# siboehm/ShallowSpeed

Measured on AMD Instinct MI355X. Metric: samples/sec (whole node), 4-layer MLP MNIST-shape, DP×PP at 1/2/4/8 GPUs, higher is better.
Workload: dtype bf16; 1 GPU; model=mlp4_mnist_784x256x256x256x10, global_batch=16384, parallelism=dp1, schedule=naive, loss=xent, mubatches=1, hipgraph=False, fp8_fwd=False, deterministic=False

## Files before the change

### csrc/bindings.cpp

```cpp

#include <torch/extension.h>

#include <ATen/cuda/CUDAContext.h>

#include <climits>
#include <optional>
#include <string>

#include "launchers.h"

namespace {

hipStream_t cur_stream() {
    return (hipStream_t)at::cuda::getCurrentCUDAStream().stream();
}

void check_bf16(const torch::Tensor& t, const char* name) {
    TORCH_CHECK(t.is_cuda(), name, " must be on GPU");
    TORCH_CHECK(t.scalar_type() == torch::kBFloat16, name, " must be bf16");
    TORCH_CHECK(t.is_contiguous(), name, " must be contiguous");
}

void check_f32(const torch::Tensor& t, const char* name) {
    TORCH_CHECK(t.is_cuda(), name, " must be on GPU");
// ... 187 lines not shown
        out = {torch::empty({M, N}, a.options().dtype(torch::kBFloat16))};
        ok = ss_gemm_nt_f8(a.data_ptr(), asc.data_ptr(), b.data_ptr(),
                           bsc.data_ptr(), bias_p, out[0].data_ptr(), M, N, K,
                           relu, cur_stream());
    }
    TORCH_CHECK(ok, "shape outside the fp8 tier: ", M, "x", N, "x", K);
    return out;
}

torch::Tensor gemm_nt_f8(torch::Tensor a, torch::Tensor asc, torch::Tensor b,
                         torch::Tensor bsc, torch::Tensor bias, bool relu) {
    return gemm_nt_f8_any(false, a, asc, b, bsc, bias, relu)[0];
}

std::vector<torch::Tensor> gemm_nt_f8_q(torch::Tensor a, torch::Tensor asc,
                                         torch::Tensor b, torch::Tensor bsc,
                                         torch::Tensor bias, bool relu) {
    return gemm_nt_f8_any(true, a, asc, b, bsc, bias, relu);
}

void wgrad_tn_256(torch::Tensor dy, torch::Tensor x, torch::Tensor gw) {
    check_bf16(dy, "dy");
    check_bf16(x, "x");
    check_f32(gw, "gw");
    const int Kb = dy.size(0), Mo = dy.size(1), N = x.size(1);
    TORCH_CHECK(x.size(0) == Kb, "batch mismatch");
    TORCH_CHECK(gw.size(0) == Mo && gw.size(1) == N, "gw shape");
    TORCH_CHECK(ss_wgrad_tn_256(dy.data_ptr(), x.data_ptr(), gw.data_ptr(),
                                Mo, N, Kb, cur_stream()),
                "shape outside the 256-tile wgrad tier");
}

void wgrad_tn(torch::Tensor dy, torch::Tensor x, torch::Tensor gw,
              torch::Tensor gb, torch::Tensor mask, int64_t split_k) {
    check_bf16(dy, "dy");
    check_bf16(x, "x");
    check_f32(gw, "gw");
    const int Kb = dy.size(0), Mo = dy.size(1), N = x.size(1);
    TORCH_CHECK(x.size(0) == Kb, "batch mismatch");
    TORCH_CHECK(gw.size(0) == Mo && gw.size(1) == N, "gw shape");
    const void* mask_p = opt_bf16(mask, "mask");
    TORCH_CHECK(!mask_p || mask.sizes() == dy.sizes(), "mask must match dy");
    void* gb_p = opt_f32(gb, "gb");
    TORCH_CHECK(!gb_p || gb.numel() == Mo, "gb size");
    ss_wgrad_tn(dy.data_ptr(), x.data_ptr(), mask_p, gw.data_ptr(), gb_p, Mo,
                N, Kb, (int)split_k, cur_stream());
}

void wgrad_tn_multi(torch::Tensor chunk_table, int64_t nchunks,
                    bool has_mask, torch::Tensor gw, torch::Tensor gb,
                    int64_t Mo, int64_t N, int64_t kb_chunk,
                    int64_t split_k) {
    check_table(chunk_table, 3, "chunk_table must be CUDA int64 [nchunks,3]");
    TORCH_CHECK(chunk_table.size(0) == nchunks,
                "chunk_table must be CUDA int64 [nchunks,3]");
    check_f32(gw, "gw");
    TORCH_CHECK(gw.size(0) == Mo && gw.size(1) == N, "gw shape");
    void* gb_p = opt_f32(gb, "gb");
    TORCH_CHECK(!gb_p || gb.numel() == Mo, "gb size");
    ss_wgrad_tn_multi(chunk_table.data_ptr(), (int)nchunks, has_mask,
                      gw.data_ptr(), gb_p, (int)Mo, (int)N, (int)kb_chunk,
                      (int)split_k, cur_stream());
}

torch::Tensor colsum(torch::Tensor dy, torch::Tensor mask) {
    check_bf16(dy, "dy");
    const void* mask_p = opt_bf16(mask, "mask");
    auto gb = torch::zeros({dy.size(1)},
                           dy.options().dtype(torch::kFloat));
    ss_colsum(dy.data_ptr(), mask_p, gb.data_ptr(), dy.size(0), dy.size(1),
              cur_stream());
    return gb;
}

torch::Tensor relu_fwd(torch::Tensor x, std::optional<torch::Tensor> out) {
    check_bf16(x, "x");
    auto y = out_like(x, out);
    ss_relu_fwd(x.data_ptr(), y.data_ptr(), x.numel(), cur_stream());
    return y;
// ... 392 lines not shown
                                 out.data_ptr(), cur_stream()),
                "shape outside the fused-MLP tier");
    return out;
}

void transpose_bf16(torch::Tensor src, torch::Tensor dst) {
    check_bf16(src, "src");
    check_bf16(dst, "dst");
    const int rows = src.size(0), cols = src.size(1);
    TORCH_CHECK(src.dim() == 2 && dst.dim() == 2 &&
                    dst.size(0) == cols && dst.size(1) == rows &&
                    rows % 64 == 0 && cols % 64 == 0,
                "transpose_bf16 needs 64-aligned 2-D shapes");
    ss_transpose_bf16(src.data_ptr(), dst.data_ptr(), rows, cols,
                      cur_stream());
}

}

PYBIND11_MODULE(TORCH_EXTENSION_NAME, m) {
    m.def("gemm_nt", &gemm_nt, "C = A @ B^T (+bias)(+relu) with optional A-mask");
    m.def("gemm_nt_256", &gemm_nt_256,
          "256-tile 8-phase GEMM (M%256==N%256==K%128==0)");
    m.def("gemm_nt_256w", &gemm_nt_256w,
          "256-tile 8-phase GEMM, 4-wave 128x128-wave-tile variant");
    m.def("wgrad_tn_256", &wgrad_tn_256,
          "256-tile 8-phase wgrad: gw += dy^T @ x (no mask/bias)");
    m.def("fp8_quantize", &fp8_quantize,
          "bf16 [R,K] -> (e4m3 u8 [R,K], e8m0 scales [K/128,R,4])");
    m.def("gemm_nt_f8", &gemm_nt_f8,
          "MX-fp8 256-tile GEMM: C=bf16(A@B^T) (+bias)(+relu)");
    m.def("gemm_nt_f8_q", &gemm_nt_f8_q,
          "MX-fp8 GEMM with FUSED output quantization -> (e4m3, scales)");
    m.def("wgrad_tn", &wgrad_tn, "gW += (dy⊙mask)^T @ x; gb += colsum (fused)");
    m.def("colsum", &colsum, "standalone column sum (bias grad)");
    m.def("wgrad_tn_multi", &wgrad_tn_multi,
          "chunked (deferred-µbatch) wgrad: one launch, many (dy,x) pairs");
    m.def("relu_fwd", &relu_fwd, py::arg("x"), py::arg("out") = py::none());
    m.def("relu_bwd", &relu_bwd, py::arg("dy"), py::arg("y"),
          py::arg("out") = py::none());
    m.def("relu_bwd_scaled", &relu_bwd_scaled,
          "dz = bf16(dy * scale) where y > 0, else +0", py::arg("dy"),
          py::arg("y"), py::arg("scale"), py::arg("out") = py::none());
    m.def("gemm_nt_dropout", &gemm_nt_dropout,
          "C = dropout(relu(A @ B^T + bias)), mask in the GEMM epilogue",
          py::arg("a"), py::arg("b"), py::arg("bias"), py::arg("key0"),
          py::arg("key1"), py::arg("step"), py::arg("layer"),
          py::arg("row_first"), py::arg("row_stride"), py::arg("thr"),
          py::arg("scale"), py::arg("fused") = true);
    m.def("dropout_fwd_", &dropout_fwd_,
          "in-place dropout of a finished post-ReLU activation");
    m.def("dropout_keep_mask", &dropout_keep_mask,
          "keep bits (bool [M][ncols]) for explicit sample ids");
    m.def("softmax_fwd", &softmax_fwd);
    m.def("softmax_bwd", &softmax_bwd);
    m.def("head_mse_bwd", &head_mse_bwd);
    m.def("head_xent_bwd", &head_xent_bwd, py::arg("probs"),
          py::arg("target"), py::arg("global_batch"),
          py::arg("out") = py::none());
    m.def("head_fwd_fused", &head_fwd_fused,
          "fused head forward: softmax(bf16(x @ w^T + b))", py::arg("x"),
          py::arg("w"), py::arg("b"), py::arg("rows_per_block") = 0);
    m.def("head_bwd_fused", &head_bwd_fused,
          "fused head backward -> (dz, dx); optional gW/gb accumulate",
          py::arg("probs"), py::arg("target"), py::arg("x"), py::arg("w_t"),
          py::arg("global_batch"), py::arg("grad_w"), py::arg("grad_b"),
          py::arg("rows_per_block") = 0,
// ... 34 lines not shown
```

### csrc/launchers.h

```cpp
#pragma once

#include <hip/hip_runtime.h>

#include <cstdint>

inline bool aligned16(const void* p) { return p && ((uintptr_t)p & 15) == 0; }

void ss_gemm_nt(const void* A, const void* B, const void* bias,
                const void* mask, void* C, int M, int N, int K, bool relu,
                hipStream_t stream);
void ss_colsum(const void* dY, const void* mask, void* gb, int M, int N,
               hipStream_t stream);

struct DropoutArgs {
    unsigned key0, key1;
    unsigned layer, step;
    unsigned row_first, row_stride;
    unsigned thr;
    float scale;
};
bool ss_gemm_nt_dropout(const void* A, const void* B, const void* bias,
                        void* C, int M, int N, int K,
                        const DropoutArgs& drop, hipStream_t stream);

bool ss_gemm_nt_256(const void* A, const void* B, const void* bias, void* C,
                    int M, int N, int K, bool relu, hipStream_t stream);
bool ss_gemm_nt_256w(const void* A, const void* B, const void* bias, void* C,
                     int M, int N, int K, bool relu, hipStream_t stream);

void ss_fp8_quantize(const void* X, void* Q, void* S, int R, int K,
                     hipStream_t stream);
bool ss_gemm_nt_f8(const void* A, const void* Asc, const void* B,
                   const void* Bsc, const void* bias, void* C, int M, int N,
                   int K, bool relu, hipStream_t stream);
bool ss_gemm_nt_f8_q(const void* A, const void* Asc, const void* B,
                     const void* Bsc, const void* bias, void* Cq, void* Cs,
                     int M, int N, int K, bool relu, hipStream_t stream);

void ss_wgrad_tn(const void* dY, const void* X, const void* mask, void* gW,
                 void* gb, int Mo, int N, int Kb, int split_k,
                 hipStream_t stream);
void ss_wgrad_tn_multi(const void* chunk_table, int nchunks, bool has_mask,
                       void* gW, void* gb, int Mo, int N, int Kb_chunk,
                       int split_k, hipStream_t stream);
bool ss_wgrad_tn_256(const void* dY, const void* X, void* gW, int Mo, int N,
                     int Kb, hipStream_t stream);

bool ss_head_fwd_fused(const void* x, const void* W, const void* bias,
                       void* probs, int M, int K, int C, int rows_per_block,
                       hipStream_t stream);
bool ss_head_bwd_fused(const void* probs, const void* target, const void* x,
                       const void* Wt, void* dz, void* dx, void* gW, void* gb,
                       int M, int K, int C, float inv_gb, int rows_per_block,
                       void* metrics, int slots, hipStream_t stream);
bool ss_head_metrics(const void* probs, const void* target, void* acc,
                     int slots, int M, int C, int kind, hipStream_t stream);

constexpr int SS_BWD_CHAIN_MAX = 8;
bool ss_bwd_chain(const void* probs, const void* target, const void* Wt_head,
                  void* dz_head, const void* const* h, const void* const* wt,
                  void* const* dz, int nlayers, void* dx, int M, int H, int C,
                  float inv_gb, int rows, int waves, int w_lds,
                  float dz_scale, hipStream_t stream);

constexpr int SS_FWD_CHAIN_MAX = 8;
bool ss_fwd_chain(const void* x, const void* const* w, const void* const* b,
                  void* const* h, int nlayers, const void* W_head,
                  const void* b_head, void* probs, int M, int K0, int H, int C,
                  int rows, int waves, int l1, hipStream_t stream);

bool ss_fused_mlp_fwd(const void* x, const void* desc, int M, int in_dim,
                      int nhidden, int cout, void* out, hipStream_t stream);

// ... 46 lines not shown
```

### csrc/wgrad.hip

```cpp

#include "common.h"
#include "launchers.h"

using gbf16 = __attribute__((address_space(1))) __bf16;
using gbf16x8 = __attribute__((address_space(1))) bf16x8;

template <int BMT, int BNT, bool HAS_MASK, int KG>
__global__ __launch_bounds__(KG * 256, BMT* BNT > 64 * 64 ? 2 : 4)
void wgrad_tn_kernel(
    const __bf16* __restrict__ dY,
    const __bf16* __restrict__ X,
    const __bf16* __restrict__ mask,
    float* __restrict__ gW,
    float* __restrict__ gb,
    int Mo, int N, int Kb, int k_per_split,
    const long* __restrict__ chunks, int nsplit) {
    constexpr int BKW = 64;
    constexpr int NMA = BMT / 16;
    constexpr int NMB = BNT / 16;
    constexpr int FM = BMT / 32;
    constexpr int FN = BNT / 32;
    constexpr int NT = KG * 256;
    constexpr int A_EL = NMA * 16 * 64;
    constexpr int B_EL = NMB * 16 * 64;
    constexpr int GRP_EL = A_EL + B_EL;
    constexpr int STAGE_F = KG * GRP_EL / 2;
    constexpr int NPASS = BMT * BNT <= STAGE_F       ? 1
                          : BMT * BNT <= 2 * STAGE_F ? 2
                                                     : 4;
    constexpr int RP = BMT / NPASS;
    static_assert(RP % 16 == 0 && RP * BNT <= STAGE_F, "epilogue band");
    static_assert(KG * 256 <= STAGE_F, "bias partials fit the staging");

    __shared__ __attribute__((aligned(16))) ushort smem[KG * GRP_EL];

    const int tid = threadIdx.x;
    const int lane = tid & 63;
    const int gtid = tid & 255;
    const int wv = __builtin_amdgcn_readfirstlane(tid >> 6);
    const int wave = wv & 3;
    const int grp = wv >> 2;
    const int wm = wave >> 1;
    const int wn = wave & 1;
    ushort* const At = smem + grp * GRP_EL;
    ushort* const Bt = At + A_EL;
    const int gx = gridDim.x, gy = gridDim.y;
    const int nwg = gx * gy * gridDim.z;
    const int hw = blockIdx.x + gx * (blockIdx.y + gy * blockIdx.z);
    const int wid = xcd_remap(hw, nwg);
    const int bidy = wid % gy;
    const int bidx = (wid / gy) % gx;
    int bidz = wid / (gy * gx);
    if (chunks) {
        const long* row = chunks + (long)(bidz / nsplit) * 3;
        dY = (const __bf16*)row[0];
        X = (const __bf16*)row[1];
        mask = (const __bf16*)row[2];
        bidz = bidz % nsplit;
    }
    const gbf16* const gdY = (const gbf16*)dY;
    const gbf16* const gX = (const gbf16*)X;
    const gbf16* const gmask = (const gbf16*)mask;
    const int m0 = bidx * BMT;
    const int n0 = bidy * BNT;
    const int kbeg = bidz * k_per_split;
    const int kend = min(Kb, kbeg + k_per_split);

    f32x4 acc[FM][FN];
#pragma unroll
    for (int i = 0; i < FM; ++i)
#pragma unroll
        for (int j = 0; j < FN; ++j) acc[i][j] = {0.f, 0.f, 0.f, 0.f};

    const int fmv = min(FM, max(0, (Mo - m0 - wm * (BMT / 2) + 15) / 16));
    const int fnv = min(FN, max(0, (N - n0 - wn * (BNT / 2) + 15) / 16));

    const bool do_db = (gb != nullptr) && (bidy == 0);
    float db_part = 0.f;

    auto swsub = [](int ksub) {
        return (ksub & ~3) | ((ksub & 1) << 1) | ((ksub >> 1) & 1);
    };
    auto baddr = [swsub](int k, int m) {
        return ((m >> 4) * 16 + swsub(k >> 2)) * 64 + (k & 3) * 16 + (m & 15);
    };

    constexpr int ELA = BKW * BMT / 256;
    constexpr int ELB = BKW * BNT / 256;
    constexpr int CA = ELA / 8, CB = ELB / 8;
    const int ska = (gtid * ELA) / BMT, sma = (gtid * ELA) % BMT;
    const int skb = (gtid * ELB) / BNT, smb = (gtid * ELB) % BNT;
    bf16x8 ra[CA], rmk[CA], rb[CB];

    auto load_chunk = [](const gbf16* p, const gbf16* base, int valid,
                         auto width_mult8) {
        bf16x8 v;
        if constexpr (decltype(width_mult8)::value) {
            v = *(const gbf16x8*)(valid > 0 ? p : base);
            return v;
        }
#pragma unroll
        for (int i = 0; i < 8; ++i) v[i] = (__bf16)0.f;
        if (valid >= 8) {
            v = *(const gbf16x8*)p;
        } else if (valid > 0) {
#pragma unroll
            for (int i = 0; i < 8; ++i) {
                const __bf16 t = p[i < valid ? i : 0];
                v[i] = i < valid ? t : (__bf16)0.f;
            }
        }
        return v;
    };
    const bool vecA = (Mo & 7) == 0, vecB = (N & 7) == 0;
    auto left_a = [&](int k0) {
        return k0 + ska < kend ? Mo - (m0 + sma) : 0;
    };
    auto left_b = [&](int k0) {
        return k0 + skb < kend ? N - (n0 + smb) : 0;
    };
    auto stage_load = [&](int k0) {
        {
            const long off = (long)(k0 + ska) * Mo + m0 + sma;
            const int left = left_a(k0);
            auto rows = [&](auto w8) {
#pragma unroll
                for (int ch = 0; ch < CA; ++ch) {
                    ra[ch] = load_chunk(gdY + off + ch * 8, gdY,
                                        left - ch * 8, w8);
                    if constexpr (HAS_MASK)
                        rmk[ch] = load_chunk(gmask + off + ch * 8, gmask,
                                             left - ch * 8, w8);
                }
            };
            if (vecA) {
                rows(std::true_type{});
            } else {
                rows(std::false_type{});
                __builtin_amdgcn_s_waitcnt(0x0F70);
            }
        }
        {
            const long off = (long)(k0 + skb) * N + n0 + smb;
            const int left = left_b(k0);
            auto rows = [&](auto w8) {
#pragma unroll
                for (int ch = 0; ch < CB; ++ch)
                    rb[ch] = load_chunk(gX + off + ch * 8, gX, left - ch * 8,
                                        w8);
            };
            if (vecB) {
                rows(std::true_type{});
            } else {
                rows(std::false_type{});
                __builtin_amdgcn_s_waitcnt(0x0F70);
            }
        }
    };
    auto stage_write = [&](int k0) {
        const int la = left_a(k0), lb = left_b(k0);
#pragma unroll
        for (int ch = 0; ch < CA; ++ch) {
            bf16x8 v = ra[ch];
            const bool in = la - ch * 8 > 0;
#pragma unroll
            for (int i = 0; i < 8; ++i) {
                bool keep = in;
                if constexpr (HAS_MASK)
                    keep = keep && bf2f(rmk[ch][i]) > 0.f;
                if (!keep) v[i] = (__bf16)0.f;
            }
            *(bf16x8*)&At[baddr(ska, sma + ch * 8)] = v;
        }
#pragma unroll
        for (int ch = 0; ch < CB; ++ch) {
            bf16x8 v = rb[ch];
            if (!(lb - ch * 8 > 0)) {
#pragma unroll
                for (int i = 0; i < 8; ++i) v[i] = (__bf16)0.f;
            }
            *(bf16x8*)&Bt[baddr(skb, smb + ch * 8)] = v;
        }
    };

    auto glds_stage = [&](const gbf16* src, ushort* img,
                          int nmt, int ld, int base_col, int gk0) {
        const int total = nmt * 16 * 8;
        const int per_wave = total / 4;
        for (int i0 = 0; i0 < per_wave; i0 += 64) {
            const int q = wave * per_wave + i0 + lane;
            const int p = q >> 3, rr = q & 7;
            const int ksub = ((p & 15) & ~3) | (((p & 15) & 1) << 1) |
                             (((p & 15) >> 1) & 1);
            const int k = ksub * 4 + (rr >> 1);
            const int m = (p >> 4) * 16 + (rr & 1) * 8;
            __builtin_amdgcn_global_load_lds(
                (gptr_t)(src + (long)(gk0 + k) * ld + base_col + m),
                (lptr_t)(img + (long)(wave * per_wave + i0) * 8), 16, 0,
                0);
        }
    };
    auto full_tile = [&](int k0) {
        return !HAS_MASK && m0 + BMT <= Mo && n0 + BNT <= N &&
               k0 + BKW <= kend;
    };

    const int lcol4 = (lane & 15) * 4;
    auto mma_step = [&](auto all_cols) {
        constexpr int FNU = decltype(all_cols)::value ? FN : 1;
#pragma unroll
        for (int kk = 0; kk < BKW / 32; ++kk) {
            const int g2 = kk * 8 + (lane >> 4) * 2;
            bf16x8 a_frag[FM], b_frag[FNU];
#pragma unroll
            for (int i = 0; i < FM; ++i) {
                const int mblk = wm * FM + i;
                bf16x4v lo = __builtin_amdgcn_ds_read_tr16_b64_v4bf16(
                    (lds_v4p)&At[(mblk * 16 + swsub(g2)) * 64 + lcol4]);
                bf16x4v hi = __builtin_amdgcn_ds_read_tr16_b64_v4bf16(
                    (lds_v4p)&At[(mblk * 16 + swsub(g2 + 1)) * 64 + lcol4]);
#pragma unroll
                for (int e = 0; e < 4; ++e) {
                    a_frag[i][e] = lo[e];
                    a_frag[i][e + 4] = hi[e];
                }
            }
#pragma unroll
            for (int j = 0; j < FNU; ++j) {
                const int nblk = wn * FN + j;
                bf16x4v lo = __builtin_amdgcn_ds_read_tr16_b64_v4bf16(
                    (lds_v4p)&Bt[(nblk * 16 + swsub(g2)) * 64 + lcol4]);
                bf16x4v hi = __builtin_amdgcn_ds_read_tr16_b64_v4bf16(
                    (lds_v4p)&Bt[(nblk * 16 + swsub(g2 + 1)) * 64 + lcol4]);
#pragma unroll
                for (int e = 0; e < 4; ++e) {
                    b_frag[j][e] = lo[e];
                    b_frag[j][e + 4] = hi[e];
                }
            }
#pragma unroll
            for (int i = 0; i < FM; ++i) {
#pragma unroll
                for (int j = 0; j < FNU; ++j)
                    acc[i][j] = __builtin_amdgcn_mfma_f32_16x16x32_bf16(
                        a_frag[i], b_frag[j], acc[i][j], 0, 0, 0);
            }
        }
    };

    const int nsteps = kend > kbeg ? (kend - kbeg + BKW - 1) / BKW : 0;
    const int niter = (nsteps + KG - 1) / KG;
    int k0 = kbeg + grp * BKW;
    if (k0 < kend && !full_tile(k0)) stage_load(k0);
    for (int it = 0; it < niter; ++it, k0 += KG * BKW) {
        const bool active = k0 < kend;
        __builtin_amdgcn_s_waitcnt(0x0F70);
        if (active) {
            if (full_tile(k0)) {
                glds_stage(gdY, At, NMA, Mo, m0, k0);
                glds_stage(gX, Bt, NMB, N, n0, k0);
            } else {
                stage_write(k0);
            }
        }
        __syncthreads();

        const int kn = k0 + KG * BKW;
        if (kn < kend && !full_tile(kn)) stage_load(kn);

        if (active) {
            if (do_db) {
                constexpr int NKQ = 256 / BMT;
                constexpr int KPT = BKW / NKQ;
                const int m = gtid % BMT, kq = gtid / BMT;
#pragma unroll
                for (int j = 0; j < KPT; ++j) {
                    const ushort u = At[baddr(kq * KPT + j, m)];
                    db_part += bf2f(*(const __bf16*)&u);
                }
            }
            if (fmv > 0 && fnv > 1)
                mma_step(std::true_type{});
            else if (fmv > 0 && fnv == 1)
                mma_step(std::false_type{});
        }
        __syncthreads();
    }

    float* const red = (float*)smem;

    if (do_db) {
        constexpr int NQ = KG * (256 / BMT);
        red[tid] = db_part;
        __syncthreads();
        if (tid < BMT && m0 + tid < Mo) {
            float s = 0.f;
#pragma unroll
            for (int qq = 0; qq < NQ; ++qq) s += red[qq * BMT + tid];
            atomicAdd(&gb[m0 + tid], s);
        }
        __syncthreads();
    }

    const int lrow = lane & 15;
    const int kch = lane >> 4;
#pragma unroll
    for (int p = 0; p < NPASS; ++p) {
#pragma unroll
        for (int g = 0; g < KG; ++g) {
            if (grp == g) {
#pragma unroll
                for (int i = 0; i < FM; ++i) {
                    const int trow = wm * (BMT / 2) + i * 16;
                    if (trow / RP != p || i >= fmv) continue;
#pragma unroll
                    for (int j = 0; j < FN; ++j) {
                        if (j >= fnv) continue;
                        const int cc = wn * (BNT / 2) + j * 16 + lrow;
#pragma unroll
                        for (int rr = 0; rr < 4; ++rr) {
                            const int ix =
                                (trow - p * RP + kch * 4 + rr) * BNT + cc;
                            if (g == 0)
                                red[ix] = acc[i][j][rr];
                            else
                                red[ix] += acc[i][j][rr];
                        }
                    }
                }
            }
            __syncthreads();
        }
        for (int ix = tid; ix < RP * BNT; ix += NT) {
            const int grow = m0 + p * RP + ix / BNT;
            const int gcol = n0 + ix % BNT;
            if (grow < Mo && gcol < N)
                atomicAdd(&gW[(long)grow * N + gcol], red[ix]);
        }
        if (p + 1 < NPASS) __syncthreads();
    }
}


namespace {

constexpr int WGRAD_KG_128 = 2;
constexpr int WGRAD_KG_64 = 4;
constexpr int WGRAD_TARGET_BLOCKS = 256;

struct WgradCfg {
    int bm, bn, kg;
};

WgradCfg wgrad_cfg(int Mo, int N, int split_k) {
    int tile = ((Mo >= 256 && N >= 512) || (Mo >= 512 && N >= 256)) ? 1 : 0;
    static const int env_big = env_int("SS_WGRAD_BIG", -1);
    static const int env_kg = env_int("SS_WGRAD_KG", -1);
    if (env_big >= 0) tile = env_big > 2 ? 1 : env_big;
    WgradCfg c;
    c.bm = tile == 1 ? 128 : 64;
    c.bn = tile == 0 ? 64 : 128;
    c.kg = tile == 0 ? WGRAD_KG_64 : WGRAD_KG_128;
    if (env_kg == 1 || env_kg == 2 || env_kg == 4) c.kg = env_kg;
    if (tile != 0 && c.kg > 2) c.kg = 2;
    if (split_k == 1) c.kg = 1;
    return c;
}

int wgrad_auto_split(int tiles, int Kb, int kg) {
    static const int env_blocks = env_int("SS_WGRAD_BLOCKS", 0);
    const int target = env_blocks > 0 ? env_blocks : WGRAD_TARGET_BLOCKS;
    int split_k = cdiv(target, tiles);
    while (split_k & (split_k - 1)) split_k &= split_k - 1;
    const int max_split = cdiv(Kb, 64 * kg);
    if (split_k > max_split) split_k = max_split;
    return split_k;
}

}

#define WGRAD_LAUNCH(BMT, BNT, HM, KGV, ...)                                \
    hipLaunchKernelGGL((wgrad_tn_kernel<BMT, BNT, HM, KGV>), grid,          \
                       dim3(KGV * 256), 0, stream, __VA_ARGS__)
#define WGRAD_BY_MASK(BMT, BNT, KGV, ...)                                   \
    do {                                                                    \
        if (has_mask) WGRAD_LAUNCH(BMT, BNT, true, KGV, __VA_ARGS__);       \
        else WGRAD_LAUNCH(BMT, BNT, false, KGV, __VA_ARGS__);               \
    } while (0)
#define WGRAD_DISPATCH(cfg, ...)                                            \
    do {                                                                    \
        if (cfg.bm == 128) {                                                \
            if (cfg.kg == 1) WGRAD_BY_MASK(128, 128, 1, __VA_ARGS__);       \
            else WGRAD_BY_MASK(128, 128, 2, __VA_ARGS__);                   \
        } else if (cfg.bn == 128) {                                         \
            if (cfg.kg == 1) WGRAD_BY_MASK(64, 128, 1, __VA_ARGS__);        \
            else WGRAD_BY_MASK(64, 128, 2, __VA_ARGS__);                    \
        } else {                                                            \
            if (cfg.kg == 1) WGRAD_BY_MASK(64, 64, 1, __VA_ARGS__);         \
            else if (cfg.kg == 2) WGRAD_BY_MASK(64, 64, 2, __VA_ARGS__);    \
            else WGRAD_BY_MASK(64, 64, 4, __VA_ARGS__);                     \
        }                                                                   \
    } while (0)

void ss_wgrad_tn(const void* dY, const void* X, const void* mask, void* gW,
                 void* gb, int Mo, int N, int Kb, int split_k,
                 hipStream_t stream) {
    if (!mask && split_k <= 0 && Mo >= 512 && N >= 512 &&
        (long)(Mo / 256) * (N / 256) >= 64) {
        static const int en = env_int("SS_WGRAD256", 1);
        if (en && ss_wgrad_tn_256(dY, X, gW, Mo, N, Kb, stream)) {
            if (gb) ss_colsum(dY, nullptr, gb, Kb, Mo, stream);
            return;
        }
    }
    const WgradCfg cfg = wgrad_cfg(Mo, N, split_k);
    if (split_k <= 0)
        split_k = wgrad_auto_split(cdiv(Mo, cfg.bm) * cdiv(N, cfg.bn), Kb,
                                   cfg.kg);
    int k_per_split = cdiv(cdiv(Kb, split_k), 64) * 64;
    split_k = cdiv(Kb, k_per_split);
    dim3 grid(cdiv(Mo, cfg.bm), cdiv(N, cfg.bn), split_k);
    const bool has_mask = mask != nullptr;
    WGRAD_DISPATCH(cfg, (const __bf16*)dY, (const __bf16*)X,
                   (const __bf16*)mask, (float*)gW, (float*)gb, Mo, N, Kb,
                   k_per_split, (const long*)nullptr, 1);
}

void ss_wgrad_tn_multi(const void* chunk_table, int nchunks, bool has_mask,
                       void* gW, void* gb, int Mo, int N, int Kb_chunk,
                       int split_k, hipStream_t stream) {
    const WgradCfg cfg = wgrad_cfg(Mo, N, split_k);
    if (split_k <= 0)
        split_k = wgrad_auto_split(
            cdiv(Mo, cfg.bm) * cdiv(N, cfg.bn) * nchunks, Kb_chunk, cfg.kg);
    int k_per_split = cdiv(cdiv(Kb_chunk, split_k), 64) * 64;
    split_k = cdiv(Kb_chunk, k_per_split);
    dim3 grid(cdiv(Mo, cfg.bm), cdiv(N, cfg.bn), split_k * nchunks);
    WGRAD_DISPATCH(cfg, (const __bf16*)nullptr, (const __bf16*)nullptr,
                   (const __bf16*)nullptr, (float*)gW, (float*)gb, Mo, N,
                   Kb_chunk, k_per_split, (const long*)chunk_table, split_k);
}
```

Baseline: 126.0 million samples/sec.

## Add double-buffered LDS staging to wgrad K loop with selectable stage count

Moves the wgrad tile body into a shared header and adds an NSTAGE template parameter. With two stages, the kernel alternates between two LDS buffer sets so the next K-step's global-to-LDS loads are issued while MFMAs run on the current set, which removes the load/compute serialization of the single-buffer loop. The stage count is exposed through the Python binding and chosen by a launcher heuristic or env var. Two stages double LDS use per block, which can lower occupancy.

```diff
diff --git a/csrc/bindings.cpp b/csrc/bindings.cpp
--- a/csrc/bindings.cpp
+++ b/csrc/bindings.cpp
@@ -243,7 +243,8 @@
 }
 
 void wgrad_tn(torch::Tensor dy, torch::Tensor x, torch::Tensor gw,
-              torch::Tensor gb, torch::Tensor mask, int64_t split_k) {
+              torch::Tensor gb, torch::Tensor mask, int64_t split_k,
+              int64_t stages) {
     check_bf16(dy, "dy");
     check_bf16(x, "x");
     check_f32(gw, "gw");
@@ -254,8 +255,9 @@
     TORCH_CHECK(!mask_p || mask.sizes() == dy.sizes(), "mask must match dy");
     void* gb_p = opt_f32(gb, "gb");
     TORCH_CHECK(!gb_p || gb.numel() == Mo, "gb size");
+    TORCH_CHECK(stages >= 0 && stages <= 2, "stages must be 0, 1 or 2");
     ss_wgrad_tn(dy.data_ptr(), x.data_ptr(), mask_p, gw.data_ptr(), gb_p, Mo,
-                N, Kb, (int)split_k, cur_stream());
+                N, Kb, (int)split_k, (int)stages, cur_stream());
 }
 
 void wgrad_tn_multi(torch::Tensor chunk_table, int64_t nchunks,
@@ -714,7 +716,11 @@
           "MX-fp8 256-tile GEMM: C=bf16(A@B^T) (+bias)(+relu)");
     m.def("gemm_nt_f8_q", &gemm_nt_f8_q,
           "MX-fp8 GEMM with FUSED output quantization -> (e4m3, scales)");
-    m.def("wgrad_tn", &wgrad_tn, "gW += (dy⊙mask)^T @ x; gb += colsum (fused)");
+    m.def("wgrad_tn", &wgrad_tn,
+          "gW += (dy⊙mask)^T @ x; gb += colsum (fused); stages = LDS "
+          "staging sets of the K loop (0 = the launcher's choice)",
+          py::arg("dy"), py::arg("x"), py::arg("gw"), py::arg("gb"),
+          py::arg("mask"), py::arg("split_k"), py::arg("stages") = 0);
     m.def("colsum", &colsum, "standalone column sum (bias grad)");
     m.def("wgrad_tn_multi", &wgrad_tn_multi,
           "chunked (deferred-µbatch) wgrad: one launch, many (dy,x) pairs");
diff --git a/csrc/launchers.h b/csrc/launchers.h
--- a/csrc/launchers.h
+++ b/csrc/launchers.h
@@ -38,7 +38,7 @@
                      int M, int N, int K, bool relu, hipStream_t stream);
 
 void ss_wgrad_tn(const void* dY, const void* X, const void* mask, void* gW,
-                 void* gb, int Mo, int N, int Kb, int split_k,
+                 void* gb, int Mo, int N, int Kb, int split_k, int stages,
                  hipStream_t stream);
 void ss_wgrad_tn_multi(const void* chunk_table, int nchunks, bool has_mask,
                        void* gW, void* gb, int Mo, int N, int Kb_chunk,
diff --git a/csrc/wgrad.hip b/csrc/wgrad.hip
--- a/csrc/wgrad.hip
+++ b/csrc/wgrad.hip
@@ -1,11 +1,33 @@
 
 #include "common.h"
 #include "launchers.h"
+#include "wgrad_dev.h"
 
-using gbf16 = __attribute__((address_space(1))) __bf16;
-using gbf16x8 = __attribute__((address_space(1))) bf16x8;
+#define WGRAD_DECODE                                                        \
+    const int gx = gridDim.x, gy = gridDim.y;                               \
+    const int nwg = gx * gy * gridDim.z;                                    \
+    const int hw = blockIdx.x + gx * (blockIdx.y + gy * blockIdx.z);        \
+    const int wid = xcd_remap(hw, nwg);                                     \
+    const int bidy = wid % gy;                                              \
+    const int bidx = (wid / gy) % gx;                                       \
+    int bidz = wid / (gy * gx);                                             \
+    if (chunks) {                                                           \
+        const long* row = chunks + (long)(bidz / nsplit) * 3;               \
+        dY = (const __bf16*)row[0];                                         \
+        X = (const __bf16*)row[1];                                          \
+        mask = (const __bf16*)row[2];                                       \
+        bidz = bidz % nsplit;                                               \
+    }                                                                       \
+    const gbf16* const gdY = (const gbf16*)dY;                              \
+    const gbf16* const gX = (const gbf16*)X;                                \
+    const gbf16* const gmask = (const gbf16*)mask;                          \
+    const int m0 = bidx * BMT;                                              \
+    const int n0 = bidy * BNT;                                              \
+    const int kbeg = bidz * k_per_split;                                    \
+    const int kend = min(Kb, kbeg + k_per_split);
+#define WGRAD_DB_OWNER bidy == 0
 
-template <int BMT, int BNT, bool HAS_MASK, int KG>
+template <int BMT, int BNT, bool HAS_MASK, int KG, int NSTAGE>
 __global__ __launch_bounds__(KG * 256, BMT* BNT > 64 * 64 ? 2 : 4)
 void wgrad_tn_kernel(
     const __bf16* __restrict__ dY,
@@ -15,331 +37,13 @@
     float* __restrict__ gb,
     int Mo, int N, int Kb, int k_per_split,
     const long* __restrict__ chunks, int nsplit) {
-    constexpr int BKW = 64;
-    constexpr int NMA = BMT / 16;
-    constexpr int NMB = BNT / 16;
-    constexpr int FM = BMT / 32;
-    constexpr int FN = BNT / 32;
-    constexpr int NT = KG * 256;
-    constexpr int A_EL = NMA * 16 * 64;
-    constexpr int B_EL = NMB * 16 * 64;
-    constexpr int GRP_EL = A_EL + B_EL;
-    constexpr int STAGE_F = KG * GRP_EL / 2;
-    constexpr int NPASS = BMT * BNT <= STAGE_F       ? 1
-                          : BMT * BNT <= 2 * STAGE_F ? 2
-                                                     : 4;
-    constexpr int RP = BMT / NPASS;
-    static_assert(RP % 16 == 0 && RP * BNT <= STAGE_F, "epilogue band");
-    static_assert(KG * 256 <= STAGE_F, "bias partials fit the staging");
-
-    __shared__ __attribute__((aligned(16))) ushort smem[KG * GRP_EL];
-
-    const int tid = threadIdx.x;
-    const int lane = tid & 63;
-    const int gtid = tid & 255;
-    const int wv = __builtin_amdgcn_readfirstlane(tid >> 6);
-    const int wave = wv & 3;
-    const int grp = wv >> 2;
-    const int wm = wave >> 1;
-    const int wn = wave & 1;
-    ushort* const At = smem + grp * GRP_EL;
-    ushort* const Bt = At + A_EL;
-    const int gx = gridDim.x, gy = gridDim.y;
-    const int nwg = gx * gy * gridDim.z;
-    const int hw = blockIdx.x + gx * (blockIdx.y + gy * blockIdx.z);
-    const int wid = xcd_remap(hw, nwg);
-    const int bidy = wid % gy;
-    const int bidx = (wid / gy) % gx;
-    int bidz = wid / (gy * gx);
-    if (chunks) {
-        const long* row = chunks + (long)(bidz / nsplit) * 3;
-        dY = (const __bf16*)row[0];
-        X = (const __bf16*)row[1];
-        mask = (const __bf16*)row[2];
-        bidz = bidz % nsplit;
-    }
-    const gbf16* const gdY = (const gbf16*)dY;
-    const gbf16* const gX = (const gbf16*)X;
-    const gbf16* const gmask = (const gbf16*)mask;
-    const int m0 = bidx * BMT;
-    const int n0 = bidy * BNT;
-    const int kbeg = bidz * k_per_split;
-    const int kend = min(Kb, kbeg + k_per_split);
-
-    f32x4 acc[FM][FN];
-#pragma unroll
-    for (int i = 0; i < FM; ++i)
-#pragma unroll
-        for (int j = 0; j < FN; ++j) acc[i][j] = {0.f, 0.f, 0.f, 0.f};
-
-    const int fmv = min(FM, max(0, (Mo - m0 - wm * (BMT / 2) + 15) / 16));
-    const int fnv = min(FN, max(0, (N - n0 - wn * (BNT / 2) + 15) / 16));
-
-    const bool do_db = (gb != nullptr) && (bidy == 0);
-    float db_part = 0.f;
-
-    auto swsub = [](int ksub) {
-        return (ksub & ~3) | ((ksub & 1) << 1) | ((ksub >> 1) & 1);
-    };
-    auto baddr = [swsub](int k, int m) {
-        return ((m >> 4) * 16 + swsub(k >> 2)) * 64 + (k & 3) * 16 + (m & 15);
-    };
-
-    constexpr int ELA = BKW * BMT / 256;
-    constexpr int ELB = BKW * BNT / 256;
-    constexpr int CA = ELA / 8, CB = ELB / 8;
-    const int ska = (gtid * ELA) / BMT, sma = (gtid * ELA) % BMT;
-    const int skb = (gtid * ELB) / BNT, smb = (gtid * ELB) % BNT;
-    bf16x8 ra[CA], rmk[CA], rb[CB];
-
-    auto load_chunk = [](const gbf16* p, const gbf16* base, int valid,
-                         auto width_mult8) {
-        bf16x8 v;
-        if constexpr (decltype(width_mult8)::value) {
-            v = *(const gbf16x8*)(valid > 0 ? p : base);
-            return v;
-        }
-#pragma unroll
-        for (int i = 0; i < 8; ++i) v[i] = (__bf16)0.f;
-        if (valid >= 8) {
-            v = *(const gbf16x8*)p;
-        } else if (valid > 0) {
-#pragma unroll
-            for (int i = 0; i < 8; ++i) {
-                const __bf16 t = p[i < valid ? i : 0];
-                v[i] = i < valid ? t : (__bf16)0.f;
-            }
-        }
-        return v;
-    };
-    const bool vecA = (Mo & 7) == 0, vecB = (N & 7) == 0;
-    auto left_a = [&](int k0) {
-        return k0 + ska < kend ? Mo - (m0 + sma) : 0;
-    };
-    auto left_b = [&](int k0) {
-        return k0 + skb < kend ? N - (n0 + smb) : 0;
-    };
-    auto stage_load = [&](int k0) {
-        {
-            const long off = (long)(k0 + ska) * Mo + m0 + sma;
-            const int left = left_a(k0);
-            auto rows = [&](auto w8) {
-#pragma unroll
-                for (int ch = 0; ch < CA; ++ch) {
-                    ra[ch] = load_chunk(gdY + off + ch * 8, gdY,
-                                        left - ch * 8, w8);
-                    if constexpr (HAS_MASK)
-                        rmk[ch] = load_chunk(gmask + off + ch * 8, gmask,
-                                             left - ch * 8, w8);
-                }
-            };
-            if (vecA) {
-                rows(std::true_type{});
-            } else {
-                rows(std::false_type{});
-                __builtin_amdgcn_s_waitcnt(0x0F70);
-            }
-        }
-        {
-            const long off = (long)(k0 + skb) * N + n0 + smb;
-            const int left = left_b(k0);
-            auto rows = [&](auto w8) {
-#pragma unroll
-                for (int ch = 0; ch < CB; ++ch)
-                    rb[ch] = load_chunk(gX + off + ch * 8, gX, left - ch * 8,
-                                        w8);
-            };
-            if (vecB) {
-                rows(std::true_type{});
-            } else {
-                rows(std::false_type{});
-                __builtin_amdgcn_s_waitcnt(0x0F70);
-            }
-        }
-    };
-    auto stage_write = [&](int k0) {
-        const int la = left_a(k0), lb = left_b(k0);
-#pragma unroll
-        for (int ch = 0; ch < CA; ++ch) {
-            bf16x8 v = ra[ch];
-            const bool in = la - ch * 8 > 0;
-#pragma unroll
-            for (int i = 0; i < 8; ++i) {
-                bool keep = in;
-                if constexpr (HAS_MASK)
-                    keep = keep && bf2f(rmk[ch][i]) > 0.f;
-                if (!keep) v[i] = (__bf16)0.f;
-            }
-            *(bf16x8*)&At[baddr(ska, sma + ch * 8)] = v;
-        }
-#pragma unroll
-        for (int ch = 0; ch < CB; ++ch) {
-            bf16x8 v = rb[ch];
-            if (!(lb - ch * 8 > 0)) {
-#pragma unroll
-                for (int i = 0; i < 8; ++i) v[i] = (__bf16)0.f;
-            }
-            *(bf16x8*)&Bt[baddr(skb, smb + ch * 8)] = v;
-        }
-    };
-
-    auto glds_stage = [&](const gbf16* src, ushort* img,
-                          int nmt, int ld, int base_col, int gk0) {
-        const int total = nmt * 16 * 8;
-        const int per_wave = total / 4;
-        for (int i0 = 0; i0 < per_wave; i0 += 64) {
-            const int q = wave * per_wave + i0 + lane;
-            const int p = q >> 3, rr = q & 7;
-            const int ksub = ((p & 15) & ~3) | (((p & 15) & 1) << 1) |
-                             (((p & 15) >> 1) & 1);
-            const int k = ksub * 4 + (rr >> 1);
-            const int m = (p >> 4) * 16 + (rr & 1) * 8;
-            __builtin_amdgcn_global_load_lds(
-                (gptr_t)(src + (long)(gk0 + k) * ld + base_col + m),
-                (lptr_t)(img + (long)(wave * per_wave + i0) * 8), 16, 0,
-                0);
-        }
-    };
-    auto full_tile = [&](int k0) {
-        return !HAS_MASK && m0 + BMT <= Mo && n0 + BNT <= N &&
-               k0 + BKW <= kend;
-    };
-
-    const int lcol4 = (lane & 15) * 4;
-    auto mma_step = [&](auto all_cols) {
-        constexpr int FNU = decltype(all_cols)::value ? FN : 1;
-#pragma unroll
-        for (int kk = 0; kk < BKW / 32; ++kk) {
-            const int g2 = kk * 8 + (lane >> 4) * 2;
-            bf16x8 a_frag[FM], b_frag[FNU];
-#pragma unroll
-            for (int i = 0; i < FM; ++i) {
-                const int mblk = wm * FM + i;
-                bf16x4v lo = __builtin_amdgcn_ds_read_tr16_b64_v4bf16(
-                    (lds_v4p)&At[(mblk * 16 + swsub(g2)) * 64 + lcol4]);
-                bf16x4v hi = __builtin_amdgcn_ds_read_tr16_b64_v4bf16(
-                    (lds_v4p)&At[(mblk * 16 + swsub(g2 + 1)) * 64 + lcol4]);
-#pragma unroll
-                for (int e = 0; e < 4; ++e) {
-                    a_frag[i][e] = lo[e];
-                    a_frag[i][e + 4] = hi[e];
-                }
-            }
-#pragma unroll
-            for (int j = 0; j < FNU; ++j) {
-                const int nblk = wn * FN + j;
-                bf16x4v lo = __builtin_amdgcn_ds_read_tr16_b64_v4bf16(
-                    (lds_v4p)&Bt[(nblk * 16 + swsub(g2)) * 64 + lcol4]);
-                bf16x4v hi = __builtin_amdgcn_ds_read_tr16_b64_v4bf16(
-                    (lds_v4p)&Bt[(nblk * 16 + swsub(g2 + 1)) * 64 + lcol4]);
-#pragma unroll
-                for (int e = 0; e < 4; ++e) {
-                    b_frag[j][e] = lo[e];
-                    b_frag[j][e + 4] = hi[e];
-                }
-            }
-#pragma unroll
-            for (int i = 0; i < FM; ++i) {
-#pragma unroll
-                for (int j = 0; j < FNU; ++j)
-                    acc[i][j] = __builtin_amdgcn_mfma_f32_16x16x32_bf16(
-                        a_frag[i], b_frag[j], acc[i][j], 0, 0, 0);
-            }
-        }
-    };
-
-    const int nsteps = kend > kbeg ? (kend - kbeg + BKW - 1) / BKW : 0;
-    const int niter = (nsteps + KG - 1) / KG;
-    int k0 = kbeg + grp * BKW;
-    if (k0 < kend && !full_tile(k0)) stage_load(k0);
-    for (int it = 0; it < niter; ++it, k0 += KG * BKW) {
-        const bool active = k0 < kend;
-        __builtin_amdgcn_s_waitcnt(0x0F70);
-        if (active) {
-            if (full_tile(k0)) {
-                glds_stage(gdY, At, NMA, Mo, m0, k0);
-                glds_stage(gX, Bt, NMB, N, n0, k0);
-            } else {
-                stage_write(k0);
-            }
-        }
-        __syncthreads();
-
-        const int kn = k0 + KG * BKW;
-        if (kn < kend && !full_tile(kn)) stage_load(kn);
-
-        if (active) {
-            if (do_db) {
-                constexpr int NKQ = 256 / BMT;
-                constexpr int KPT = BKW / NKQ;
-                const int m = gtid % BMT, kq = gtid / BMT;
-#pragma unroll
-                for (int j = 0; j < KPT; ++j) {
-                    const ushort u = At[baddr(kq * KPT + j, m)];
-                    db_part += bf2f(*(const __bf16*)&u);
-                }
-            }
-            if (fmv > 0 && fnv > 1)
-                mma_step(std::true_type{});
-            else if (fmv > 0 && fnv == 1)
-                mma_step(std::false_type{});
-        }
-        __syncthreads();
-    }
-
-    float* const red = (float*)smem;
-
-    if (do_db) {
-        constexpr int NQ = KG * (256 / BMT);
-        red[tid] = db_part;
-        __syncthreads();
-        if (tid < BMT && m0 + tid < Mo) {
-            float s = 0.f;
-#pragma unroll
-            for (int qq = 0; qq < NQ; ++qq) s += red[qq * BMT + tid];
-            atomicAdd(&gb[m0 + tid], s);
-        }
-        __syncthreads();
-    }
-
-    const int lrow = lane & 15;
-    const int kch = lane >> 4;
-#pragma unroll
-    for (int p = 0; p < NPASS; ++p) {
-#pragma unroll
-        for (int g = 0; g < KG; ++g) {
-            if (grp == g) {
-#pragma unroll
-                for (int i = 0; i < FM; ++i) {
-                    const int trow = wm * (BMT / 2) + i * 16;
-                    if (trow / RP != p || i >= fmv) continue;
-#pragma unroll
-                    for (int j = 0; j < FN; ++j) {
-                        if (j >= fnv) continue;
-                        const int cc = wn * (BNT / 2) + j * 16 + lrow;
-#pragma unroll
-                        for (int rr = 0; rr < 4; ++rr) {
-                            const int ix =
-                                (trow - p * RP + kch * 4 + rr) * BNT + cc;
-                            if (g == 0)
-                                red[ix] = acc[i][j][rr];
-                            else
-                                red[ix] += acc[i][j][rr];
-                        }
-                    }
-                }
-            }
-            __syncthreads();
-        }
-        for (int ix = tid; ix < RP * BNT; ix += NT) {
-            const int grow = m0 + p * RP + ix / BNT;
-            const int gcol = n0 + ix % BNT;
-            if (grow < Mo && gcol < N)
-                atomicAdd(&gW[(long)grow * N + gcol], red[ix]);
-        }
-        if (p + 1 < NPASS) __syncthreads();
-    }
+    __shared__ __attribute__((aligned(16)))
+    ushort smem[NSTAGE * wgrad_set_el<BMT, BNT, KG>()];
+#define WGRAD_TILE_HERE
+#include "wgrad_dev.h"
 }
+#undef WGRAD_DECODE
+#undef WGRAD_DB_OWNER
 
 
 namespace {
@@ -377,11 +81,27 @@
     return split_k;
 }
 
+int wgrad_stages(const WgradCfg& cfg, int Mo, int N, bool has_mask,
+                 int stages) {
+    if (stages == 1 || stages == 2) return stages;
+    static const int env_stages = env_int("SS_WGRAD_STAGES", 0);
+    if (env_stages == 1 || env_stages == 2) return env_stages;
+    return !has_mask && cfg.kg > 1 && Mo >= cfg.bm && N >= cfg.bn ? 2 : 1;
+}
+
 }
 
 #define WGRAD_LAUNCH(BMT, BNT, HM, KGV, ...)                                \
-    hipLaunchKernelGGL((wgrad_tn_kernel<BMT, BNT, HM, KGV>), grid,          \
-                       dim3(KGV * 256), 0, stream, __VA_ARGS__)
+    do {                                                                    \
+        if (stages == 2)                                                    \
+            hipLaunchKernelGGL((wgrad_tn_kernel<BMT, BNT, HM, KGV, 2>),     \
+                               grid, dim3(KGV * 256), 0, stream,            \
+                               __VA_ARGS__);                                \
+        else                                                                \
+            hipLaunchKernelGGL((wgrad_tn_kernel<BMT, BNT, HM, KGV, 1>),     \
+                               grid, dim3(KGV * 256), 0, stream,            \
+                               __VA_ARGS__);                                \
+    } while (0)
 #define WGRAD_BY_MASK(BMT, BNT, KGV, ...)                                   \
     do {                                                                    \
         if (has_mask) WGRAD_LAUNCH(BMT, BNT, true, KGV, __VA_ARGS__);       \
@@ -403,7 +123,7 @@
     } while (0)
 
 void ss_wgrad_tn(const void* dY, const void* X, const void* mask, void* gW,
-                 void* gb, int Mo, int N, int Kb, int split_k,
+                 void* gb, int Mo, int N, int Kb, int split_k, int stages,
                  hipStream_t stream) {
     if (!mask && split_k <= 0 && Mo >= 512 && N >= 512 &&
         (long)(Mo / 256) * (N / 256) >= 64) {
@@ -421,6 +141,7 @@
     split_k = cdiv(Kb, k_per_split);
     dim3 grid(cdiv(Mo, cfg.bm), cdiv(N, cfg.bn), split_k);
     const bool has_mask = mask != nullptr;
+    stages = wgrad_stages(cfg, Mo, N, has_mask, stages);
     WGRAD_DISPATCH(cfg, (const __bf16*)dY, (const __bf16*)X,
                    (const __bf16*)mask, (float*)gW, (float*)gb, Mo, N, Kb,
                    k_per_split, (const long*)nullptr, 1);
@@ -436,6 +157,7 @@
     int k_per_split = cdiv(cdiv(Kb_chunk, split_k), 64) * 64;
     split_k = cdiv(Kb_chunk, k_per_split);
     dim3 grid(cdiv(Mo, cfg.bm), cdiv(N, cfg.bn), split_k * nchunks);
+    const int stages = 1;
     WGRAD_DISPATCH(cfg, (const __bf16*)nullptr, (const __bf16*)nullptr,
                    (const __bf16*)nullptr, (float*)gW, (float*)gb, Mo, N,
                    Kb_chunk, k_per_split, (const long*)chunk_table, split_k);
diff --git a/csrc/wgrad_dev.h b/csrc/wgrad_dev.h
--- /dev/null
+++ b/csrc/wgrad_dev.h
@@ -0,0 +1,384 @@
+#ifndef SS_WGRAD_DEV_H
+#define SS_WGRAD_DEV_H
+
+#include "common.h"
+
+using gbf16 = __attribute__((address_space(1))) __bf16;
+using gbf16x8 = __attribute__((address_space(1))) bf16x8;
+
+template <int BMT, int BNT, int KG>
+constexpr int wgrad_set_el() {
+    return KG * (BMT + BNT) * 64;
+}
+
+template <class Issue, class Compute>
+__device__ __forceinline__ void wgrad_two_sets(ushort* __restrict__ cur,
+                                               ushort* __restrict__ nxt,
+                                               Issue issue, Compute compute) {
+    issue(nxt);
+    compute(cur);
+}
+
+#endif
+
+#ifdef WGRAD_TILE_HERE
+#undef WGRAD_TILE_HERE
+{
+    static_assert(NSTAGE == 1 || NSTAGE == 2, "staging depth");
+    constexpr int BKW = 64;
+    constexpr int NMA = BMT / 16;
+    constexpr int NMB = BNT / 16;
+    constexpr int FM = BMT / 32;
+    constexpr int FN = BNT / 32;
+    constexpr int NT = KG * 256;
+    constexpr int A_EL = NMA * 16 * 64;
+    constexpr int B_EL = NMB * 16 * 64;
+    constexpr int GRP_EL = A_EL + B_EL;
+    constexpr int STAGE_F = KG * GRP_EL / 2;
+    constexpr int NPASS = BMT * BNT <= STAGE_F       ? 1
+                          : BMT * BNT <= 2 * STAGE_F ? 2
+                                                     : 4;
+    constexpr int RP = BMT / NPASS;
+    static_assert(RP % 16 == 0 && RP * BNT <= STAGE_F, "epilogue band");
+    static_assert(KG * 256 <= STAGE_F, "bias partials fit the staging");
+
+    static_assert(KG * GRP_EL == wgrad_set_el<BMT, BNT, KG>(), "set size");
+
+    const int tid = threadIdx.x;
+    const int lane = tid & 63;
+    const int gtid = tid & 255;
+    const int wv = __builtin_amdgcn_readfirstlane(tid >> 6);
+    const int wave = wv & 3;
+    const int grp = wv >> 2;
+    const int wm = wave >> 1;
+    const int wn = wave & 1;
+    using img_t = std::conditional_t<NSTAGE == 1, ushort* const, ushort*>;
+    img_t At = smem + grp * GRP_EL;
+    img_t Bt = At + A_EL;
+    WGRAD_DECODE
+
+    f32x4 acc[FM][FN];
+#pragma unroll
+    for (int i = 0; i < FM; ++i)
+#pragma unroll
+        for (int j = 0; j < FN; ++j) acc[i][j] = {0.f, 0.f, 0.f, 0.f};
+
+    const int fmv = min(FM, max(0, (Mo - m0 - wm * (BMT / 2) + 15) / 16));
+    const int fnv = min(FN, max(0, (N - n0 - wn * (BNT / 2) + 15) / 16));
+
+    const bool do_db = (gb != nullptr) && (WGRAD_DB_OWNER);
+    float db_part = 0.f;
+
+    auto swsub = [](int ksub) {
+        return (ksub & ~3) | ((ksub & 1) << 1) | ((ksub >> 1) & 1);
+    };
+    auto baddr = [swsub](int k, int m) {
+        return ((m >> 4) * 16 + swsub(k >> 2)) * 64 + (k & 3) * 16 + (m & 15);
+    };
+
+    constexpr int ELA = BKW * BMT / 256;
+    constexpr int ELB = BKW * BNT / 256;
+    constexpr int CA = ELA / 8, CB = ELB / 8;
+    const int ska = (gtid * ELA) / BMT, sma = (gtid * ELA) % BMT;
+    const int skb = (gtid * ELB) / BNT, smb = (gtid * ELB) % BNT;
+    bf16x8 ra[CA], rmk[CA], rb[CB];
+
+    auto load_chunk = [](const gbf16* p, const gbf16* base, int valid,
+                         auto width_mult8) {
+        bf16x8 v;
+        if constexpr (decltype(width_mult8)::value) {
+            v = *(const gbf16x8*)(valid > 0 ? p : base);
+            return v;
+        }
+#pragma unroll
+        for (int i = 0; i < 8; ++i) v[i] = (__bf16)0.f;
+        if (valid >= 8) {
+            v = *(const gbf16x8*)p;
+        } else if (valid > 0) {
+#pragma unroll
+            for (int i = 0; i < 8; ++i) {
+                const __bf16 t = p[i < valid ? i : 0];
+                v[i] = i < valid ? t : (__bf16)0.f;
+            }
+        }
+        return v;
+    };
+    const bool vecA = (Mo & 7) == 0, vecB = (N & 7) == 0;
+    auto left_a = [&](int k0) {
+        return k0 + ska < kend ? Mo - (m0 + sma) : 0;
+    };
+    auto left_b = [&](int k0) {
+        return k0 + skb < kend ? N - (n0 + smb) : 0;
+    };
+    auto stage_load = [&](int k0) {
+        {
+            const long off = (long)(k0 + ska) * Mo + m0 + sma;
+            const int left = left_a(k0);
+            auto rows = [&](auto w8) {
+#pragma unroll
+                for (int ch = 0; ch < CA; ++ch) {
+                    ra[ch] = load_chunk(gdY + off + ch * 8, gdY,
+                                        left - ch * 8, w8);
+                    if constexpr (HAS_MASK)
+                        rmk[ch] = load_chunk(gmask + off + ch * 8, gmask,
+                                             left - ch * 8, w8);
+                }
+            };
+            if (vecA) {
+                rows(std::true_type{});
+            } else {
+                rows(std::false_type{});
+                __builtin_amdgcn_s_waitcnt(0x0F70);
+            }
+        }
+        {
+            const long off = (long)(k0 + skb) * N + n0 + smb;
+            const int left = left_b(k0);
+            auto rows = [&](auto w8) {
+#pragma unroll
+                for (int ch = 0; ch < CB; ++ch)
+                    rb[ch] = load_chunk(gX + off + ch * 8, gX, left - ch * 8,
+                                        w8);
+            };
+            if (vecB) {
+                rows(std::true_type{});
+            } else {
+                rows(std::false_type{});
+                __builtin_amdgcn_s_waitcnt(0x0F70);
+            }
+        }
+    };
+    auto stage_write = [&](int k0) {
+        const int la = left_a(k0), lb = left_b(k0);
+#pragma unroll
+        for (int ch = 0; ch < CA; ++ch) {
+            bf16x8 v = ra[ch];
+            const bool in = la - ch * 8 > 0;
+#pragma unroll
+            for (int i = 0; i < 8; ++i) {
+                bool keep = in;
+                if constexpr (HAS_MASK)
+                    keep = keep && bf2f(rmk[ch][i]) > 0.f;
+                if (!keep) v[i] = (__bf16)0.f;
+            }
+            *(bf16x8*)&At[baddr(ska, sma + ch * 8)] = v;
+        }
+#pragma unroll
+        for (int ch = 0; ch < CB; ++ch) {
+            bf16x8 v = rb[ch];
+            if (!(lb - ch * 8 > 0)) {
+#pragma unroll
+                for (int i = 0; i < 8; ++i) v[i] = (__bf16)0.f;
+            }
+            *(bf16x8*)&Bt[baddr(skb, smb + ch * 8)] = v;
+        }
+    };
+
+    auto glds_stage = [&](const gbf16* src, ushort* img,
+                          int nmt, int ld, int base_col, int gk0) {
+        const int total = nmt * 16 * 8;
+        const int per_wave = total / 4;
+        for (int i0 = 0; i0 < per_wave; i0 += 64) {
+            const int q = wave * per_wave + i0 + lane;
+            const int p = q >> 3, rr = q & 7;
+            const int ksub = ((p & 15) & ~3) | (((p & 15) & 1) << 1) |
+                             (((p & 15) >> 1) & 1);
+            const int k = ksub * 4 + (rr >> 1);
+            const int m = (p >> 4) * 16 + (rr & 1) * 8;
+            __builtin_amdgcn_global_load_lds(
+                (gptr_t)(src + (long)(gk0 + k) * ld + base_col + m),
+                (lptr_t)(img + (long)(wave * per_wave + i0) * 8), 16, 0,
+                0);
+        }
+    };
+    auto full_tile = [&](int k0) {
+        return !HAS_MASK && m0 + BMT <= Mo && n0 + BNT <= N &&
+               k0 + BKW <= kend;
+    };
+
+    const int lcol4 = (lane & 15) * 4;
+    auto mma_step = [&](auto all_cols, const ushort* Ai = nullptr,
+                        const ushort* Bi = nullptr) {
+        const ushort* const Ar = NSTAGE == 1 ? At : Ai;
+        const ushort* const Br = NSTAGE == 1 ? Bt : Bi;
+        constexpr int FNU = decltype(all_cols)::value ? FN : 1;
+#pragma unroll
+        for (int kk = 0; kk < BKW / 32; ++kk) {
+            const int g2 = kk * 8 + (lane >> 4) * 2;
+            bf16x8 a_frag[FM], b_frag[FNU];
+#pragma unroll
+            for (int i = 0; i < FM; ++i) {
+                const int mblk = wm * FM + i;
+                bf16x4v lo = __builtin_amdgcn_ds_read_tr16_b64_v4bf16(
+                    (lds_v4p)&Ar[(mblk * 16 + swsub(g2)) * 64 + lcol4]);
+                bf16x4v hi = __builtin_amdgcn_ds_read_tr16_b64_v4bf16(
+                    (lds_v4p)&Ar[(mblk * 16 + swsub(g2 + 1)) * 64 + lcol4]);
+#pragma unroll
+                for (int e = 0; e < 4; ++e) {
+                    a_frag[i][e] = lo[e];
+                    a_frag[i][e + 4] = hi[e];
+                }
+            }
+#pragma unroll
+            for (int j = 0; j < FNU; ++j) {
+                const int nblk = wn * FN + j;
+                bf16x4v lo = __builtin_amdgcn_ds_read_tr16_b64_v4bf16(
+                    (lds_v4p)&Br[(nblk * 16 + swsub(g2)) * 64 + lcol4]);
+                bf16x4v hi = __builtin_amdgcn_ds_read_tr16_b64_v4bf16(
+                    (lds_v4p)&Br[(nblk * 16 + swsub(g2 + 1)) * 64 + lcol4]);
+#pragma unroll
+                for (int e = 0; e < 4; ++e) {
+                    b_frag[j][e] = lo[e];
+                    b_frag[j][e + 4] = hi[e];
+                }
+            }
+#pragma unroll
+            for (int i = 0; i < FM; ++i) {
+#pragma unroll
+                for (int j = 0; j < FNU; ++j)
+                    acc[i][j] = __builtin_amdgcn_mfma_f32_16x16x32_bf16(
+                        a_frag[i], b_frag[j], acc[i][j], 0, 0, 0);
+            }
+        }
+    };
+
+    const int nsteps = kend > kbeg ? (kend - kbeg + BKW - 1) / BKW : 0;
+    const int niter = (nsteps + KG - 1) / KG;
+    int k0 = kbeg + grp * BKW;
+    if constexpr (NSTAGE == 1) {
+        if (k0 < kend && !full_tile(k0)) stage_load(k0);
+        for (int it = 0; it < niter; ++it, k0 += KG * BKW) {
+            const bool active = k0 < kend;
+            __builtin_amdgcn_s_waitcnt(0x0F70);
+            if (active) {
+                if (full_tile(k0)) {
+                    glds_stage(gdY, At, NMA, Mo, m0, k0);
+                    glds_stage(gX, Bt, NMB, N, n0, k0);
+                } else {
+                    stage_write(k0);
+                }
+            }
+            __syncthreads();
+
+            const int kn = k0 + KG * BKW;
+            if (kn < kend && !full_tile(kn)) stage_load(kn);
+
+            if (active) {
+                if (do_db) {
+                    constexpr int NKQ = 256 / BMT;
+                    constexpr int KPT = BKW / NKQ;
+                    const int m = gtid % BMT, kq = gtid / BMT;
+#pragma unroll
+                    for (int j = 0; j < KPT; ++j) {
+                        const ushort u = At[baddr(kq * KPT + j, m)];
+                        db_part += bf2f(*(const __bf16*)&u);
+                    }
+                }
+                if (fmv > 0 && fnv > 1)
+                    mma_step(std::true_type{});
+                else if (fmv > 0 && fnv == 1)
+                    mma_step(std::false_type{});
+            }
+            __syncthreads();
+        }
+    } else {
+        constexpr int SET_EL = KG * GRP_EL;
+        ushort* const A0 = At;
+        auto issue = [&](int k, ushort* Ai) {
+            if (full_tile(k)) {
+                glds_stage(gdY, Ai, NMA, Mo, m0, k);
+                glds_stage(gX, Ai + A_EL, NMB, N, n0, k);
+            } else {
+                stage_load(k);
+            }
+        };
+        if (k0 < kend) issue(k0, A0);
+        for (int it = 0; it < niter; ++it, k0 += KG * BKW) {
+            const bool active = k0 < kend;
+            At = A0 + (it & 1) * SET_EL;
+            Bt = At + A_EL;
+            __builtin_amdgcn_s_waitcnt(0x0F70);
+            if (active && !full_tile(k0)) stage_write(k0);
+            __syncthreads();
+
+            const int kn = k0 + KG * BKW;
+            wgrad_two_sets(
+                At, A0 + ((it & 1) ^ 1) * SET_EL,
+                [&](ushort* An) {
+                    if (kn < kend) issue(kn, An);
+                },
+                [&](const ushort* Ai) {
+                    if (!active) return;
+                    if (do_db) {
+                        constexpr int NKQ = 256 / BMT;
+                        constexpr int KPT = BKW / NKQ;
+                        const int m = gtid % BMT, kq = gtid / BMT;
+#pragma unroll
+                        for (int j = 0; j < KPT; ++j) {
+                            const ushort u = Ai[baddr(kq * KPT + j, m)];
+                            db_part += bf2f(*(const __bf16*)&u);
+                        }
+                    }
+                    if (fmv > 0 && fnv > 1)
+                        mma_step(std::true_type{}, Ai, Ai + A_EL);
+                    else if (fmv > 0 && fnv == 1)
+                        mma_step(std::false_type{}, Ai, Ai + A_EL);
+                });
+        }
+        __syncthreads();
+    }
+
+    float* const red = (float*)smem;
+
+    if (do_db) {
+        constexpr int NQ = KG * (256 / BMT);
+        red[tid] = db_part;
+        __syncthreads();
+        if (tid < BMT && m0 + tid < Mo) {
+            float s = 0.f;
+#pragma unroll
+            for (int qq = 0; qq < NQ; ++qq) s += red[qq * BMT + tid];
+            atomicAdd(&gb[m0 + tid], s);
+        }
+        __syncthreads();
+    }
+
+    const int lrow = lane & 15;
+    const int kch = lane >> 4;
+#pragma unroll
+    for (int p = 0; p < NPASS; ++p) {
+#pragma unroll
+        for (int g = 0; g < KG; ++g) {
+            if (grp == g) {
+#pragma unroll
+                for (int i = 0; i < FM; ++i) {
+                    const int trow = wm * (BMT / 2) + i * 16;
+                    if (trow / RP != p || i >= fmv) continue;
+#pragma unroll
+                    for (int j = 0; j < FN; ++j) {
+                        if (j >= fnv) continue;
+                        const int cc = wn * (BNT / 2) + j * 16 + lrow;
+#pragma unroll
+                        for (int rr = 0; rr < 4; ++rr) {
+                            const int ix =
+                                (trow - p * RP + kch * 4 + rr) * BNT + cc;
+                            if (g == 0)
+                                red[ix] = acc[i][j][rr];
+                            else
+                                red[ix] += acc[i][j][rr];
+                        }
+                    }
+                }
+            }
+            __syncthreads();
+        }
+        for (int ix = tid; ix < RP * BNT; ix += NT) {
+            const int grow = m0 + p * RP + ix / BNT;
+            const int gcol = n0 + ix % BNT;
+            if (grow < Mo && gcol < N)
+                atomicAdd(&gW[(long)grow * N + gcol], red[ix]);
+        }
+        if (p + 1 < NPASS) __syncthreads();
+    }
+}
+#endif
```

Measured after the change: 133.1 million samples/sec (median of 6 runs). 1.06x the previous value.
